# sash-a/hrl_pybullet_envs

Measured on AMD Instinct MI355X. Metric: env-steps/sec, AntGatherBulletEnv-v0 @4096 envs, 1/2/4/8 MI355X, higher is better.
Workload: dtype f32; 1 GPU; AntGatherBulletEnv-v0, 4096 envs per GPU, U(-1,1) actions pre-generated on device, auto-reset, max_episode_steps 2000; envs_per_gpu=4096, global_envs=4096, parallelism=one GPU, one process, no collective

## Files before the change

### hrl_pybullet_envs_amd/csrc/step_core.h

```cpp
#pragma once
#include <math.h>
#include <stdint.h>

#include <utility>

#ifdef HRL_EMU
#define HRL_DEV inline
#define HRL_PIN_VGPR(x) ((void)0)
#define HRL_PIN_INT(x) ((void)0)
#define HRL_PIN_SCALAR(x) ((void)0)
#else
#define HRL_DEV __device__ __forceinline__
#define HRL_PIN_VGPR(x) asm volatile("" : "+v"(x))
#define HRL_PIN_INT(x) asm volatile("" : "+s"(x))
#define HRL_PIN_SCALAR(x) asm volatile("" : "+s"(x))
#endif


namespace hrl {

constexpr int NJ = 8;
constexpr int MAXC = 12;
constexpr int MAXR = 44;
constexpr int MAXB = NJ + MAXC;
// ... 1315 lines not shown
        }
        x.reg(lane).ud = d < 6 ? v : 0.f;
        if (lane < 16) L.ustar[lane] = d < 6 ? v : 0.f;
        float ax_[3], ay_[3], az_[3];
        quat_axes(q[3], q[4], q[5], q[6], ax_, ay_, az_);
#pragma unroll
        for (int k = 0; k < 3; ++k) { L.XYZ[k] = ax_[k]; L.XYZ[3 + k] = ay_[k]; L.XYZ[6 + k] = az_[k]; }
    });
    int nC = 0;
    auto corner = [&](int lane, bool on, int f, int item) {
        CornerHit h; h.ok = false; h.dist = 0.f; h.n[0] = h.n[1] = 0.f; h.n[2] = 1.f; h.c[0] = h.c[1] = h.c[2] = 0.f; h.surf = f;
        if (on) {
            float sx = (lane & 1) ? he : -he, sy = (lane & 2) ? he : -he, sz = (lane & 4) ? he : -he;
#pragma unroll
            for (int k = 0; k < 3; ++k) h.c[k] = fma_(sz, L.XYZ[6 + k], fma_(sy, L.XYZ[3 + k], sx * L.XYZ[k]));
            const float p[3] = {q[0] + h.c[0], q[1] + h.c[1], q[2] + h.c[2]};
            if (item >= 0) {
                const float ix = L.items[2 * item], iy = L.items[2 * item + 1];
                const float lo[3] = {ix - ITEM_HALF, iy - ITEM_HALF, ITEM_Z - ITEM_HALF}, hi[3] = {ix + ITEM_HALF, iy + ITEM_HALF, ITEM_Z + ITEM_HALF};
                h.dist = sphere_vs_box(p, 0.f, lo, hi, h.n); h.surf = surf_item(item);
            } else if (f == 0) h.dist = p[2] - c.ground_z;
            else {
                h.n[0] = L.planes[f - 1][0]; h.n[1] = L.planes[f - 1][1]; h.n[2] = L.planes[f - 1][2];
                h.dist = dot3(h.n, p) - L.planes[f - 1][3];
            }
            h.ok = h.dist < c.cdist;
        }
        return h;
    };
    auto keep = [&](int base) {
        return [&L, base](int, int rank, const CornerHit &h) {
            const int i = base + rank;
            if (i < MAXC) {
#pragma unroll
                for (int k = 0; k < 3; ++k) { L.cr[i][k] = h.c[k]; L.cdir[0][i][k] = h.n[k]; }
                L.cdist_[i] = h.dist; L.csurf[i] = h.surf;
            }
        };
    };
    {
        int cnt = x.each_compact([&](int lane) { return corner(lane, (lane >> 3) < 1 + c.n_planes, lane >> 3, -1); }, keep(nC), [&](int, const CornerHit &) {});
        nC += cnt;
        if (nC > cap) nC = cap;
    }
    if (items_on) {
        const float R = 0.35f * 1.7320508f + ITEM_HALF + c.cdist + 0.02f;
        unsigned long long near = x.each_ballot([&](int lane) {
            return (lane < c.n_food + c.n_poison) & (fabsf(q[0] - L.items[2 * lane]) < R) & (fabsf(q[1] - L.items[2 * lane + 1]) < R);
        });
        const unsigned long long near0 = near;
        while (near) {
            int it[4];
#pragma unroll
            for (int k = 0; k < 4; ++k) {
                it[k] = -1;
                if (near) { it[k] = (int)__builtin_ctzll(near); near &= near - 1; }
            }
            int cnt = x.each_compact(
                [&](int lane) {
                    const int slot = lane >> 3;
                    const int item = slot == 0 ? it[0] : (slot == 1 ? it[1] : (slot == 2 ? it[2] : (slot == 3 ? it[3] : -1)));
                    return corner(lane, item >= 0, 0, item);
                },
                keep(nC), [&](int, const CornerHit &) {});
            nC += cnt;
            if (nC > cap) nC = cap;
        }
        x.refresh();
#pragma unroll 1
        for (int ib = 0; ib < 64; ib += 32) {
        unsigned near32 = (unsigned)(near0 >> ib);
        while (near32) {
            const unsigned group = near32;
#pragma unroll
            for (int k = 0; k < 8; ++k) near32 &= near32 - 1;
            int cnt = x.each_compact(
                [&](int lane) {
                    const int slot = lane >> 3;
                    unsigned m = group;
#pragma unroll
                    for (int k = 0; k < 7; ++k) m = k < slot ? (m & (m - 1)) : m;
                    const int item = m ? ib + (int)__builtin_ctz(m) : -1;
                    CornerHit h; h.ok = false; h.dist = 0.f; h.n[0] = h.n[1] = 0.f; h.n[2] = 1.f; h.c[0] = h.c[1] = h.c[2] = 0.f; h.surf = 0;
                    if (item >= 0) {
                        const float ix = L.items[2 * item], iy = L.items[2 * item + 1];
                        const float pc[3] = {(lane & 1) ? ix + ITEM_HALF : ix - ITEM_HALF, (lane & 2) ? iy + ITEM_HALF : iy - ITEM_HALF,
                                             (lane & 4) ? ITEM_Z + ITEM_HALF : ITEM_Z - ITEM_HALF};
                        const float d[3] = {pc[0] - q[0], pc[1] - q[1], pc[2] - q[2]};
                        const float l[3] = {dot3(d, &L.XYZ[0]), dot3(d, &L.XYZ[3]), dot3(d, &L.XYZ[6])}, blo[3] = {-he, -he, -he}, bhi[3] = {he, he, he};
                        float nl[3];
                        h.dist = sphere_vs_box(l, 0.f, blo, bhi, nl); h.surf = surf_item(item);
#pragma unroll
                        for (int k = 0; k < 3; ++k) {
                            const float nw = fma_(nl[2], L.XYZ[6 + k], fma_(nl[1], L.XYZ[3 + k], nl[0] * L.XYZ[k]));
                            h.n[k] = -nw; h.c[k] = fma_(-h.dist, nw, d[k]);
                        }
                        h.ok = h.dist < c.cdist;
                    }
                    return h;
                },
                keep(nC), [&](int, const CornerHit &) {});
            nC += cnt;
            if (nC > cap) nC = cap;
        }
        }
    }
    x.each([&](int lane) {
        if (lane < nC) { const float n[3] = {L.cdir[0][lane][0], L.cdir[0][lane][1], L.cdir[0][lane][2]}; store_contact_frame(L, lane, n); }
    });
    x.each([&](int lane) {
        LaneRegs &g = x.reg(lane);
        g.fn = -1;
        if (lane >= 3 * nC) return;
        const int ci = lane < nC ? lane : (lane - nC) >> 1, which = lane < nC ? 0 : 1 + ((lane - nC) & 1);
        const float r[3] = {L.cr[ci][0], L.cr[ci][1], L.cr[ci][2]};
        const float d[3] = {L.cdir[which][ci][0], L.cdir[which][ci][1], L.cdir[which][ci][2]};
        float J[6], B[16];
#pragma unroll
        for (int k = 0; k < 16; ++k) B[k] = 0.f;
        cross3(J, r, d);
#pragma unroll
        for (int k = 0; k < 3; ++k) { J[3 + k] = d[k]; B[k] = J[k] / I; B[3 + k] = d[k] / m; }
        const float dist = L.cdist_[ci];
#pragma unroll
        for (int k = 0; k < 6; ++k) g.Jb[k] = J[k];
        g.Jh = 0.f; g.Ja = 0.f; g.jslot = 6 | (6 << 8); g.mu = which == 0 ? 0.f : c.mu;
#pragma unroll
        for (int k = 0; k < 16; ++k) L.Bt[lane][k] = B[k];
        g.bias = which == 0 ? (dist > 0.f ? dist : c.erp_c * dist) * c.inv_h : 0.f;
        g.fn = which == 0 ? -1 : ci; g.lam = 0.f; g.lo = 0.f; g.hi = which == 0 ? 1e30f : 0.f;
    });
    pgs_solve<MAXC>(x, c, 0, nC, false, false);
    x.each([&](int lane) { if (lane < 16) L.u[lane] = x.reg(lane).ud; });
    x.stamp(10);
    x.each([&](int lane) { phase_integrate(c, L, q, qn, lane); });
    x.stamp(11);
    return nC;
}


HRL_DEV void quat_to_rpy(const float *qq, float *rpy) {
    float x = qq[0], y = qq[1], z = qq[2], w = qq[3];
    float sarg = -2.f * (x * z - w * y);
    const float hp = 1.5707963267948966f;
    if (sarg <= -0.99999f) { rpy[0] = 0.f; rpy[1] = -hp; rpy[2] = 2.f * atan2_spec(x, -y); }
    else if (sarg >= 0.99999f) { rpy[0] = 0.f; rpy[1] = hp; rpy[2] = 2.f * atan2_spec(-x, y); }
    else {
        float sqx = x * x, sqy = y * y, sqz = z * z, sqw = w * w;
        rpy[0] = atan2_spec(2.f * (y * z + w * x), ((sqw - sqx) - sqy) + sqz);
        rpy[1] = asin_spec(sarg);
        rpy[2] = atan2_spec(2.f * (x * y + w * z), ((sqw + sqx) - sqy) - sqz);
    }
}
HRL_DEV float wrap_angle(float a) {
    const float two_pi = 6.283185307179586f, pi = 3.141592653589793f;
    if (!(fabsf(a) < two_pi)) a = fmodf(a, two_pi);
    if (a < 0.f) a += two_pi;
    if (a >= two_pi) a -= two_pi;
    if (a > pi) a = a - two_pi;
    if (a < -pi) a = a + two_pi;
    return a;
}
HRL_DEV int quadrant(float x, float y) {
    if (x >= 0.f && y >= 0.f) return 1;
    if (x >= 0.f && y <= 0.f) return 4;
    if (x <= 0.f && y >= 0.f) return 2;
    if (x <= 0.f && y <= 0.f) return 3;
    return -1;
}
HRL_DEV bool inf_intersection(float x1, float y1, float x2, float y2, float x3, float y3, float x4, float y4, float *px, float *py) {
    float d = (x1 - x2) * (y3 - y4) - (y1 - y2) * (x3 - x4);
    if (d == 0.f) return false;
    *px = ((x1 * y2 - y1 * x2) * (x3 - x4) - (x1 - x2) * (x3 * y4 - y3 * x4)) / d;
    *py = ((x1 * y2 - y1 * x2) * (y3 - y4) - (y1 - y2) * (x3 * y4 - y3 * x4)) / d;
    return true;
}
HRL_DEV int orientation(float px, float py, float qx, float qy, float rx, float ry) {
    float val = ((qy - py) * (rx - qx)) - ((qx - px) * (ry - qy));
    return val > 0.f ? 1 : (val < 0.f ? 2 : 0);
}
HRL_DEV bool on_segment(float px, float py, float qx, float qy, float rx, float ry) {
    return (qx <= fmaxf(px, rx)) && (qx >= fminf(px, rx)) && (qy <= fmaxf(py, ry)) && (qy >= fminf(py, ry));
}
HRL_DEV bool segment_intersection(float p1x, float p1y, float q1x, float q1y, float p2x, float p2y, float q2x, float q2y) {
    int o1 = orientation(p1x, p1y, q1x, q1y, p2x, p2y), o2 = orientation(p1x, p1y, q1x, q1y, q2x, q2y);
    int o3 = orientation(p2x, p2y, q2x, q2y, p1x, p1y), o4 = orientation(p2x, p2y, q2x, q2y, q1x, q1y);
    if (o1 != o2 && o3 != o4) return true;
    if (o1 == 0 && on_segment(p1x, p1y, p2x, p2y, q1x, q1y)) return true;
    if (o2 == 0 && on_segment(p1x, p1y, q2x, q2y, q1x, q1y)) return true;
    if (o3 == 0 && on_segment(p2x, p2y, p1x, p1y, q2x, q2y)) return true;
    if (o4 == 0 && on_segment(p2x, p2y, q1x, q1y, q2x, q2y)) return true;
    return false;
}
HRL_DEV void maze_line(int l, float *a) {
    const float T[7][4] = {{5, 9, -5, 9}, {5, 9, 5, -9}, {-5, -9, -5, 9}, {-5, -9, 5, -9}, {1, 2, 1, -2}, {-5, -2, -5, 2}, {-5, -2, 1, -2}};
#pragma unroll
    for (int k = 0; k < 4; ++k) {
        float v = T[0][k];
#pragma unroll
        for (int i = 1; i < 7; ++i) v = (l == i) ? T[i][k] : v;
        a[k] = v;
    }
}

HRL_DEV void flag_goal(const DevCfg &c, uint32_t ep, uint32_t k, float *gx, float *gy) {
    for (uint32_t a = 0; a < 64; ++a) {
        uint32_t r[4];
        philox4x32(c, 0, ep, (4u << 16) | k, a, r);
        *gx = -c.flag_size / 2.f + c.flag_size * u01(r[0]); *gy = -c.flag_size / 2.f + c.flag_size * u01(r[1]);
        if (!(sqrtf(*gx * *gx + *gy * *gy) < 0.5f)) break;
    }
}

HRL_DEV void flag_close_goal(const DevCfg &c, long long env, uint32_t ep, uint32_t k, float rx, float ry, float *gx, float *gy) {
    const float wb = c.flag_size / 2.f, half = c.flag_mtd / 2.f;
    for (uint32_t a = 0; a < 64; ++a) {
        uint32_t r[4];
        philox4x32(c, env, ep, (5u << 16) | (k & 0xffffu), a, r);
        *gx = (c.tol + (half - c.tol) * u01(r[0])) * ((r[2] & 1u) ? 1.f : -1.f) + rx;
        *gy = (c.tol + (half - c.tol) * u01(r[1])) * ((r[3] & 1u) ? 1.f : -1.f) + ry;
        if (-wb < *gx && *gx < wb && -wb < *gy && *gy < wb) break;
    }
}

HRL_DEV void flag_set_target_state(WaveLds &L, float gx, float gy, float px, float py) {
    const float dx = gx - px, dy = gy - py, nrm = sqrtf(dx * dx + dy * dy);
    L.items[HRL_FLAG_START_OFF] = px; L.items[HRL_FLAG_START_OFF + 1] = py; L.items[HRL_FLAG_SQDIST_OFF] = nrm * nrm;
}

HRL_DEV float wall_sensor_bin(const DevCfg &c, float rx, float ry, float yaw, int i, bool arena) {
    const float half_pi = 1.5707963267948966f;
    float phi;
    if (c.span_is_2pi) phi = half_pi + yaw + ((float)(i + 1) / (float)c.n_bins) * c.sensor_span;
    else phi = half_pi + yaw + ((float)i / (float)(c.n_bins - 1)) * c.sensor_span;
    const float svx = rx + c.sensor_range * cos_spec(phi), svy = ry + c.sensor_range * sin_spec(phi);
    const int sq = quadrant(svx - rx, svy - ry);
    float best = 0.f;
    for (int l = 0; l < (arena ? 4 : 7); ++l) {
        float a[4], px, py;
        if (arena) {
            const float hx = c.world_sx / 2.f, hy = c.world_sy / 2.f;
            a[0] = l < 2 ? hx : -hx; a[1] = l < 2 ? hy : -hy;
            a[2] = (l == 0 || l == 2) ? -hx : hx; a[3] = (l == 0) ? hy : ((l == 1) ? -hy : ((l == 2) ? hy : -hy));
        } else maze_line(l, a);
        if (!inf_intersection(rx, ry, svx, svy, a[0], a[1], a[2], a[3], &px, &py)) continue;
        const float ddx = rx - px, ddy = ry - py, dist = sqrtf(ddx * ddx + ddy * ddy);
        if (dist > c.sensor_range) continue;
        if (sq != quadrant(px - rx, py - ry)) continue;
        const float val = 1.f - dist / c.sensor_range;
        if (val > best) best = val;
    }
    return best;
}

template <class X>
HRL_DEV void maze_target(X &x, const DevCfg &c, WaveLds &L, float *tx, float *ty) {
    const unsigned ti = (unsigned)x.uniform(L.aux[3]);
    const int k = ti < (unsigned)HRL_MAX_TARGETS ? (int)ti : 0;
    *tx = c.targets[k][0]; *ty = c.targets[k][1];
}

template <int KIND>
HRL_DEV void phase_calc_state(const DevCfg &c, WaveLds &L, int lane, bool use_feet, bool with_centroid, float mtx, float mty) {
    const float *qp = L.st, *qv = L.st + 15;
    float rpy[3];
    quat_to_rpy(qp + 3, rpy);
    float tx = c.walk_tx, ty = c.walk_ty;
    if (KIND == 5) {
        if (c.flag_mtd > 0.f || c.flag_manual) { tx = L.items[0]; ty = L.items[1]; }
        else flag_goal(c, (uint32_t)L.aux[2], (uint32_t)L.aux[3] & 0xffffu, &tx, &ty);
    }
    if (KIND == 2 || KIND == 4) { tx = mtx; ty = mty; }
    if (KIND == 5) { L.red[4] = tx; L.red[5] = ty; }
    float cx = qp[0], cy = qp[1];
    if (with_centroid) {
        float sx = 0.f, sy = 0.f;
#pragma unroll
        for (int l = 0; l < 4; ++l) {
            sx += (0.5f * L.ph[l][0] + 0.5f * (L.ph[l][0] + L.pa[l][0])) + 0.5f * (L.pa[l][0] + L.tip[l][0]);
            sy += (0.5f * L.ph[l][1] + 0.5f * (L.ph[l][1] + L.pa[l][1])) + 0.5f * (L.pa[l][1] + L.tip[l][1]);
        }
        const float np_ = (float)(13 + c.centroid_n_static);
        cx = ((13.f * qp[0] + sx) + c.centroid_sx) / np_;
        cy = ((13.f * qp[1] + sy) + c.centroid_sy) / np_;
    }
    const float dx = tx - cx, dy = ty - cy;
    float sin_ang = 0.f, cos_ang = 0.f, wtd = 0.f;
    if (KIND != 1) {
        const float theta = atan2_spec(dy, dx), ang = theta - rpy[2];
        wtd = sqrtf(dy * dy + dx * dx); sin_ang = sin_spec(ang); cos_ang = cos_spec(ang);
    }
    const float cs = cos_spec(-rpy[2]), sn = sin_spec(-rpy[2]);
    const float vx = cs * qv[0] - sn * qv[1], vy = sn * qv[0] + cs * qv[1], vz = qv[2];
    int nlim = 0;
    float mine = 0.f;
#pragma unroll
    for (int j = 0; j < NJ; ++j) {
        const float rel = (qp[7 + j] - c.jmid[j]) * c.jscale[j];
        if (fabsf(rel) > 0.99f) ++nlim;
        mine = (lane == 8 + 2 * j) ? rel : mine;
        mine = (lane == 9 + 2 * j) ? 0.1f * qv[6 + j] : mine;
    }
    mine = (lane == 0) ? qp[2] - L.st[30] : mine;
    mine = (lane == 1) ? sin_ang : mine;
    mine = (lane == 2) ? cos_ang : mine;
    mine = (lane == 3) ? 0.3f * vx : mine;
    mine = (lane == 4) ? 0.3f * vy : mine;
    mine = (lane == 5) ? 0.3f * vz : mine;
    mine = (lane == 6) ? rpy[0] : mine;
    mine = (lane == 7) ? rpy[1] : mine;
    if (lane >= 24 && lane < 28) {
        const int l = lane - 24;
        mine = (use_feet && ((L.aux[1] >> (28 + l)) & 1)) ? 1.f : 0.f;
    }
    if (lane < 28) L.s28[lane] = clampf(mine, -5.f, 5.f);
    L.scal[3] = wtd; L.scal[4] = rpy[2]; L.scal[5] = (float)nlim; L.scal[6] = cx; L.scal[7] = cy;
}

HRL_DEV void respawn_item(const DevCfg &c, long long env, uint32_t index, uint32_t purpose, int item, float ax, float ay, float *px, float *py) {
    const float sxw = c.world_sx - 1.f, syw = c.world_sy - 1.f;
    for (uint32_t a = 0; a < 64; ++a) {
        uint32_t r[4];
        philox4x32(c, env, index, (purpose << 16) | (uint32_t)item, a, r);
        *px = u01(r[0]) * sxw - sxw / 2.f; *py = u01(r[1]) * syw - syw / 2.f;
        const float dx = ax - *px, dy = ay - *py;
        if (!(sqrtf(dx * dx + dy * dy) < c.spacing)) break;
    }
}

HRL_DEV void phase_items(const DevCfg &c, WaveLds &L, int lane, long long env, bool pickups, int n_contacts) {
    const int n = c.n_food + c.n_poison;
    float rew = 0.f, bin = -1.f, inten = 0.f;
    if (lane < n) {
        const float rx = L.st[0], ry = L.st[1], yaw = L.scal[4];
        float ix = L.items[2 * lane], iy = L.items[2 * lane + 1];
        float dx = ix - rx, dy = iy - ry, d2 = dx * dx + dy * dy;
        if (pickups && c.coll_dist > 0.f && d2 < c.coll_dist) {
            rew = lane < c.n_food ? 1.f : -1.f;
            if (c.respawn) respawn_item(c, env, (uint32_t)L.aux[1], 0u, lane, rx, ry, &ix, &iy);
            else { ix = 100.f; iy = 0.f; }
            L.items[2 * lane] = ix; L.items[2 * lane + 1] = iy;
            dx = ix - rx; dy = iy - ry; d2 = dx * dx + dy * dy;
        }
        if (!c.use_sensor) inten = d2;
        else if (d2 != d2) bin = -2.f;
        else if (!(d2 > c.sensor_range)) {
            const float half_span = c.sensor_span * 0.5f, bin_res = c.sensor_span / (float)c.n_bins;
            const float angle = wrap_angle(atan2_spec(iy - ry, ix - rx) - yaw);
            if (fabsf(angle) <= half_span) {
                int b = (int)((angle + half_span) / bin_res);
                if (b >= c.n_bins) b = c.n_bins - 1;
                bin = (float)b; inten = 1.0f - d2 / c.sensor_range;
            }
        }
        if (pickups && !(c.coll_dist > 0.f)) {
            int hits = 0;
            for (int i = 0; i < n_contacts; ++i) hits += L.csurf[i] == surf_item(lane) ? 1 : 0;
            rew = (lane < c.n_food ? 1.f : -1.f) * (float)hits;
        }
    }
    L.irew[lane] = rew; L.ibin[lane] = bin; L.iint[lane] = inten;
}

HRL_DEV void phase_items_contact_move(const DevCfg &c, WaveLds &L, int lane, long long env) {
    if (lane >= c.n_food + c.n_poison) return;
    const int hits = (int)fabsf(L.irew[lane]);
    if (hits > 0) {
        float ix = 100.f, iy = 0.f;
        if (c.respawn) respawn_item(c, env, (uint32_t)L.aux[1], 0u, lane | ((hits - 1) << c.item_shift), L.st[0], L.st[1], &ix, &iy);
        L.items[2 * lane] = ix; L.items[2 * lane + 1] = iy;
    }
}

template <int KIND>
HRL_DEV void phase_pack_obs(const DevCfg &c, WaveLds &L, int lane , float mtx, float mty) {
    if (lane >= c.obs_dim) return;
    float v = 0.f;
    if (KIND == 0) v = L.st[lane];
    else if (KIND == 5) {
        if (lane < 28) v = L.s28[lane];
        else v = wall_sensor_bin(c, L.st[0], L.st[1], L.scal[4], lane - 28, true);
    }
    else if (KIND == 4) {
        if (lane < 29) v = L.st[lane];
        else if (lane < 29 + c.n_bins) v = wall_sensor_bin(c, L.st[0], L.st[1], L.scal[4], lane - 29, false);
        else if (lane == 29 + 3 * c.n_bins) v = (float)L.aux[0] * 0.001f;
    }
    else if (KIND == 3) {
        if (lane < 8) v = L.s28[lane];
    } else if (lane < 26) v = L.s28[lane == 0 ? 0 : lane + 2];
    const int nb = (KIND == 3) ? 8 : 26;
    if ((KIND == 1 || KIND == 3) && lane >= nb && c.use_sensor) {
        const int b = lane - nb, type = b / c.n_bins, bin = b - type * c.n_bins;
        const int k0 = type ? c.n_food : 0, k1 = type ? c.n_food + c.n_poison : c.n_food;
        float best = 0.f;
        bool bad = false;
#pragma unroll
        for (int k = 0; k < 16; ++k) {
            const bool mine = (k >= k0) & (k < k1);
            const bool take = mine & (L.ibin[k] == (float)bin) & (L.iint[k] > best);
            best = take ? L.iint[k] : best;
            bad = bad | (mine & (L.ibin[k] == -2.f));
        }
#pragma unroll 1
        for (int k = 16; k < k1; ++k) {
            const bool mine = k >= k0;
            const bool take = mine & (L.ibin[k] == (float)bin) & (L.iint[k] > best);
            best = take ? L.iint[k] : best;
            bad = bad | (mine & (L.ibin[k] == -2.f));
        }
        v = bad ? __builtin_nanf("") : best;
    }
    if ((KIND == 1 || KIND == 3) && lane >= nb && !c.use_sensor) {
        const int mf = c.n_food < c.n_bins ? c.n_food : c.n_bins;
        const int b = lane - nb, type = b >= 2 * mf, bb = type ? b - 2 * mf : b, want = bb >> 1, comp = bb & 1;
        const int k0 = type ? c.n_food : 0, k1 = type ? c.n_food + c.n_poison : c.n_food;
        bool bad = false;
        for (int i = k0; i < k1; ++i) {
            int rank = 0;
            for (int j = k0; j < k1; ++j) rank += (L.iint[j] < L.iint[i] || (L.iint[j] == L.iint[i] && j < i)) ? 1 : 0;
            if (rank == want) v = L.items[2 * i + comp];
            bad = bad | (L.iint[i] != L.iint[i]);
        }
        if (bad && want < (k1 - k0)) v = __builtin_nanf("");
    }
    if (KIND == 2 && lane >= 26) {
        const float rx = L.st[0], ry = L.st[1], yaw = L.scal[4];
        const float tx = mtx, ty = mty;
        const int ntar = c.sense_target ? c.n_bins : 2;
        if (lane < 26 + ntar) {
            const int i = lane - 26;
            if (!c.sense_target) {
                const float vx = tx - rx, vy = ty - ry;
                if (c.target_encoding == 0) { const float n = sqrtf(vx * vx + vy * vy); v = i == 0 ? vx / n : vy / n; }
                else { const float a = atan2_spec(vy, vx) - yaw; v = i == 0 ? sin_spec(a) : cos_spec(a); }
            } else {
                const float wtd = L.scal[3];
                bool vis = !(wtd > c.sensor_range);
                for (int l = 4; l < 7 && vis; ++l) { float a[4]; maze_line(l, a); if (segment_intersection(rx, ry, tx, ty, a[0], a[1], a[2], a[3])) vis = false; }
                if (vis) {
                    const float angle = wrap_angle(atan2_spec(ty - ry, tx - rx) - yaw), half_span = c.sensor_span * 0.5f;
                    if (fabsf(angle) <= half_span) {
                        int b = (int)((angle + half_span) / (c.sensor_span / (float)c.n_bins));
                        if (b >= c.n_bins) b = c.n_bins - 1;
                        if (b == i) v = 1.0f - wtd / c.sensor_range;
                    }
                }
            }
        } else v = wall_sensor_bin(c, rx, ry, yaw, lane - 26 - ntar, false);
    }
    L.obs[lane] = v;
    if (!isfinite(v)) L.flags[0] = 1;
}

HRL_DEV void phase_point_state(const DevCfg &c, WaveLds &L, int lane) {
    const float *qp = L.st, *qv = L.st + 15;
    float rpy[3];
    quat_to_rpy(qp + 3, rpy);
    const float theta = atan2_spec(0.f - qp[1], 0.f - qp[0]), a = theta - rpy[2];
    const float cs = cos_spec(-rpy[2]), sn = sin_spec(-rpy[2]);
    const float vx = cs * qv[0] - sn * qv[1], vy = sn * qv[0] + cs * qv[1], vz = qv[2];
    float mine = qp[2] - 1.f;
    mine = (lane == 1) ? sin_spec(a) : mine;
    mine = (lane == 2) ? cos_spec(a) : mine;
    mine = (lane == 3) ? 0.3f * vx : mine;
    mine = (lane == 4) ? 0.3f * vy : mine;
    mine = (lane == 5) ? 0.3f * vz : mine;
    mine = (lane == 6) ? rpy[0] : mine;
    mine = (lane == 7) ? rpy[1] : mine;
    if (lane < 8) L.s28[lane] = mine;
    L.scal[3] = 0.f; L.scal[4] = rpy[2]; L.scal[5] = 0.f;
    (void)c;
}

template <int KIND, class X>
HRL_DEV void compute_obs(X &x, const DevCfg &c, long long env, bool step_mode, int n_contacts = 0) {
    WaveLds &L = x.lds();
    const bool centroid = (KIND == 0 || KIND == 2 || KIND == 4 || KIND == 5);
    if (centroid) {
        x.each([&](int lane) { if (lane < 16) L.q[0][lane] = lane < 15 ? L.st[lane] : 0.f; });
        x.each([&](int lane) { phase_kin_ankle<true>(c, L, x.reg(lane), L.q[0], lane); });
    }
    float mtx = 0.f, mty = 0.f;
    if (KIND == 2 || KIND == 4) maze_target(x, c, L, &mtx, &mty);
    x.each([&](int lane) { if (lane < 4) L.flags[lane] = 0; });
    if (KIND == 3) x.each([&](int lane) { phase_point_state(c, L, lane); });
    else {
        const bool feet = KIND == 2 || KIND == 5;
        x.each([&](int lane) { phase_calc_state<KIND>(c, L, lane, feet, centroid, mtx, mty); });
    }
    x.stamp(21);
    if (KIND == 1 || KIND == 3) x.each([&](int lane) { phase_items(c, L, lane, env, step_mode, n_contacts); });
    x.stamp(22);
#pragma unroll 1
    for (int o = 0; o < c.obs_dim; o += 64) x.each([&](int lane) { phase_pack_obs<KIND>(c, L, lane + o, mtx, mty); });
    if ((KIND == 1 || KIND == 3) && step_mode && !(c.coll_dist > 0.f)) x.each([&](int lane) { phase_items_contact_move(c, L, lane, env); });
}


template <int KIND, class X>
HRL_DEV void reset_env(X &x, const DevCfg &c, long long env) {
    WaveLds &L = x.lds();
    float ptx = c.walk_tx, pty = c.walk_ty;
    if (KIND == 2 || KIND == 4 || KIND == 5) {
        if (x.uniform(L.aux[2]) > 0) {
            if (KIND == 5) {
                if (c.flag_mtd > 0.f || c.flag_manual) { ptx = L.items[0]; pty = L.items[1]; }
                else flag_goal(c, (uint32_t)L.aux[2], (uint32_t)L.aux[3] & 0xffffu, &ptx, &pty);
            } else maze_target(x, c, L, &ptx, &pty);
        }
        x.each([](int) {});
    }
    x.each([&](int lane) {
        const uint32_t ep = (uint32_t)L.aux[2];
        if (lane < 32) {
            float v = 0.f;
            if (lane == 6) v = 1.f;
            if (KIND == 3) { if (lane == 2) v = 0.5f; if (lane == 30) v = 1.f; }
            else {
                float z0 = 0.75f;
                if (KIND == 2 || KIND == 4 || KIND == 5) { z0 = c.start_pos[2]; if (lane == 0) v = c.start_pos[0]; if (lane == 1) v = c.start_pos[1]; }
                if (lane == 2 || lane == 30) v = z0;
                if (lane >= 7 && lane < 15) {
                    const int j = lane - 7;
                    uint32_t r[4];
                    philox4x32(c, env, ep, (2u << 16) | (uint32_t)(j >> 2), 0u, r);
                    const uint32_t rr = (j & 3) == 0 ? r[0] : ((j & 3) == 1 ? r[1] : ((j & 3) == 2 ? r[2] : r[3]));
                    v = -0.1f + 0.2f * u01(rr);
                }
            }
            L.st[lane] = v;
        } else if (KIND == 1 || KIND == 3) {
            const int i = lane - 32;
            if (i < 16) {
                float px = 0.f, py = 0.f;
                if (i < c.n_food + c.n_poison) respawn_item(c, env, ep, 1u, i, 0.f, 0.f, &px, &py);
                L.items[2 * i] = px; L.items[2 * i + 1] = py;
            }
        } else if (KIND == 5 && c.flag_path_on) {
            const int w = lane - 32;
            if (c.flag_manual) {
                if (w == 0) L.items[0] = ptx;
                if (w == 1) L.items[1] = pty;
                if (w >= HRL_FLAG_PENDING_OFF) L.items[w] = 0.f;
            } else {
                float gx = 0.f, gy = 0.f;
                if (w == 0) {
                    if (c.flag_mtd > 0.f) flag_close_goal(c, env, ep + 1u, 1u, c.start_pos[0], c.start_pos[1], &gx, &gy);
                    else flag_goal(c, ep + 1u, 1u, &gx, &gy);
                    flag_set_target_state(L, gx, gy, c.start_pos[0], c.start_pos[1]);
                    L.items[0] = c.flag_mtd > 0.f ? gx : 0.f; L.items[1] = c.flag_mtd > 0.f ? gy : 0.f;
                    L.items[HRL_FLAG_SQDIST_OFF + 1] = 0.f;
                } else if (w >= HRL_FLAG_PENDING_OFF) L.items[w] = 0.f;
            }
        }
        if (lane < 16) L.u[lane] = 0.f;
        if (lane < 8) L.tau[lane] = 0.f;
        if (lane == 63 && KIND == 5) L.aux[3] = (int)((c.flag_manual ? 0u : 1u) | ((uint32_t)L.aux[3] & 0x7fff0000u));
        if (lane == 63 && (KIND == 2 || KIND == 4)) {
            uint32_t r[4];
            philox4x32(c, env, ep, (3u << 16), 0u, r);
            L.aux[3] = (int)(r[0] % (uint32_t)c.n_targets);
        }
    });
    if ((KIND == 1 || KIND == 3 || KIND == 5) && c.items_stride > 32)
        x.each([&](int lane) {
            const uint32_t ep = (uint32_t)L.aux[2];
            const int i = 16 + lane;
            if (i < HRL_MAX_ITEMS) {
                float px = 0.f, py = 0.f;
                if ((KIND == 1 || KIND == 3) && i < c.n_food + c.n_poison) respawn_item(c, env, ep, 1u, i, 0.f, 0.f, &px, &py);
                L.items[2 * i] = px; L.items[2 * i + 1] = py;
            }
        });
    x.each([&](int lane) {
        if (lane == 0) L.aux[0] = 0;
        if (lane == 1 && (KIND == 2 || KIND == 5)) L.aux[1] = L.aux[1] & 0x0fffffff;
        if (lane == 2) L.aux[2] = L.aux[2] + 1;
    });
    compute_obs<KIND>(x, c, env, false);
    x.each([&](int lane) {
        if (lane != 31) return;
        float pot = 0.f;
        if (KIND == 0) pot = -L.scal[3] / c.dt;
        if (KIND == 2 || KIND == 4 || KIND == 5) {
            float cx = L.scal[6], cy = L.scal[7];
            if (KIND != 5) { const float np_ = (float)(13 + c.centroid_n_static); cx = cx - (13.f * c.start_pos[0]) / np_; cy = cy - (13.f * c.start_pos[1]) / np_; }
            const float dx = ptx - cx, dy = pty - cy;
            pot = -sqrtf(dy * dy + dx * dx) / c.dt;
        }
        L.st[31] = pot;
    });
}

template <class X>
HRL_DEV void load_env(X &x, const DevBufs &b, const DevCfg &c, int e, bool with_actions) {
    WaveLds &L = x.lds();
    x.each([&](int lane) {
        if (lane < 32) L.st[lane] = b.state[(size_t)e * 32 + lane];
        else { const float v = b.items ? b.items[(size_t)e * c.items_stride + (lane - 32)] : 0.f; L.items[lane - 32] = v; L.items0[lane - 32] = v; }
#pragma unroll 1
        for (int o = 32; o < c.items_stride; o += 64)
            if (o + lane < c.items_stride) L.items[o + lane] = b.items ? b.items[(size_t)e * c.items_stride + (o + lane)] : 0.f;
        if (lane < 4) L.aux[lane] = b.aux[(size_t)e * 4 + lane];
        if (lane < 8) L.act[lane] = (with_actions && lane < c.act_dim) ? b.actions[(size_t)e * c.act_dim + lane] : 0.f;
        if (lane >= 8 && lane < 16) { L.jlim[0][lane - 8] = c.jlo[lane - 8]; L.jlim[1][lane - 8] = c.jhi[lane - 8]; }
        if (lane >= 16 && lane < 32) { const int f = (lane - 16) >> 2, k = lane & 3; L.planes[f][k] = k < 3 ? c.plane_n[f][k] : c.plane_d[f]; }
    });
}
template <class X>
HRL_DEV void store_env(X &x, const DevBufs &b, const DevCfg &c, int e) {
    WaveLds &L = x.lds();
    x.each([&](int lane) {
        if (lane < 32) b.state[(size_t)e * 32 + lane] = L.st[lane];
        else if (b.items) {
            const float v = L.items[lane - 32];
            if (float_bits(v) != float_bits(L.items0[lane - 32])) b.items[(size_t)e * c.items_stride + (lane - 32)] = v;
        }
#pragma unroll 1
        for (int o = 32; o < c.items_stride; o += 64)
            if (b.items && o + lane < c.items_stride) b.items[(size_t)e * c.items_stride + (o + lane)] = L.items[o + lane];
        if (lane < 4) b.aux[(size_t)e * 4 + lane] = L.aux[lane];
        if (lane < c.obs_dim) b.obs[(size_t)e * c.obs_dim + lane] = L.obs[lane];
#pragma unroll 1
        for (int o = 64; o < c.obs_dim; o += 64)
            if (o + lane < c.obs_dim) b.obs[(size_t)e * c.obs_dim + (o + lane)] = L.obs[o + lane];
    });
}

template <int KIND, class X>
HRL_DEV void reset_entry(X &x, const DevBufs &b, const DevCfg &c, int e) {
    if (b.mask && !b.mask[e]) return;
    load_env(x, b, c, e, false);
    reset_env<KIND>(x, c, c.env_id_offset + e);
    store_env(x, b, c, e);
}

template <int KIND, class X>
HRL_DEV void observe_entry(X &x, const DevBufs &b, const DevCfg &c, int e) {
    if (b.mask && !b.mask[e]) return;
    WaveLds &L = x.lds();
    load_env(x, b, c, e, false);
    compute_obs<KIND>(x, c, c.env_id_offset + e, false);
    x.each([&](int lane) {
#pragma unroll 1
        for (int o = 0; o < c.obs_dim; o += 64)
            if (o + lane < c.obs_dim) b.obs[(size_t)e * c.obs_dim + (o + lane)] = L.obs[o + lane];
    });
}

template <class X>
HRL_DEV void set_goals_entry(X &x, const DevBufs &b, const DevCfg &c, int e, const float *goals_xy, int n_goals, uint8_t *ok) {
    if (b.mask && !b.mask[e]) return;
    WaveLds &L = x.lds();
    const long long env = c.env_id_offset + e;
    load_env(x, b, c, e, false);
    if (n_goals > 0) {
        x.each([&](int lane) {
#pragma unroll 1
            for (int w = lane; w < c.items_stride; w += 64)
                if (w >= HRL_FLAG_PENDING_OFF) {
                    const int k = (w - HRL_FLAG_PENDING_OFF) >> 1, comp = w & 1;
                    L.items[w] = k < n_goals ? goals_xy[((size_t)e * n_goals + k) * 2 + comp] : 0.f;
                }
            if (lane == 63) L.aux[3] = (int)(((uint32_t)n_goals & 0xffffu) | ((uint32_t)L.aux[3] & 0xffff0000u));
        });
    }
    x.each([&](int lane) {
        if (lane != 0) return;
        const uint32_t a3 = (uint32_t)L.aux[3];
        uint32_t cur = a3 & 0xffffu;
        int good = 1;
        float gx = L.items[0], gy = L.items[1];
        if (c.flag_mtd > 0.f) {
            cur = (cur + 1u) & 0xffffu;
            flag_close_goal(c, env, (uint32_t)L.aux[2], cur, L.st[0], L.st[1], &gx, &gy);
        } else if (!c.flag_manual) {
            if (cur >= (uint32_t)c.flag_max_targets) good = 0; else cur += 1u;
        } else if (cur == 0u) good = 0;
        else { cur -= 1u; gx = L.items[HRL_FLAG_PENDING_OFF + 2 * cur]; gy = L.items[HRL_FLAG_PENDING_OFF + 1 + 2 * cur]; }
        if (good) {
            if (!c.flag_manual && !(c.flag_mtd > 0.f)) flag_goal(c, (uint32_t)L.aux[2], cur, &gx, &gy);
            else { L.items[0] = gx; L.items[1] = gy; }
            if (c.flag_path_on) flag_set_target_state(L, gx, gy, L.st[0], L.st[1]);
            L.aux[3] = (int)(cur | (a3 & 0x7fff0000u));
        }
        if (ok) ok[e] = (uint8_t)good;
    });
    compute_obs<5>(x, c, env, false);
    store_env(x, b, c, e);
}

template <int KIND, class X>
HRL_DEV void write_contacts(X &x, const DevCfg &c, float *rec, const float *q0, int n_contacts, int nL) {
    const WaveLds &L = x.lds();
    x.each([&](int lane) {
        float v0 = 0.f, v1 = 0.f, v2 = 0.f, v3 = 0.f;
        const int nR = nL + 3 * n_contacts;
        if (lane == 0) { v0 = (float)n_contacts; v1 = (float)nL; v2 = (float)nR; v3 = c.h; }
        else if (lane < 3) {
            for (int k = 0; k < nL; ++k) {
                const int j = (L.ljoint[k] & 7) - 4 * (lane - 1);
                const float f = L.lsign[k] * L.lamf[k];
                v0 = j == 0 ? f : v0; v1 = j == 1 ? f : v1; v2 = j == 2 ? f : v2; v3 = j == 3 ? f : v3;
            }
        } else if (lane == 3) {
            int held = 0, neg = 0;
            for (int k = 0; k < nL; ++k) { const int bit = 1 << (L.ljoint[k] & 7); held |= bit; neg |= L.lsign[k] < 0.f ? bit : 0; }
            v0 = (float)held; v1 = (float)neg;
        } else {
            const int m = lane - 4, i = m / 5, w = m - 5 * i;
            if (i < n_contacts) {
                if (w == 0) { v0 = L.cr[i][0] + q0[0]; v1 = L.cr[i][1] + q0[1]; v2 = L.cr[i][2] + q0[2]; v3 = L.cdist_[i]; }
                else if (w < 4) {
                    const int d = w - 1;
                    v0 = L.cdir[d][i][0]; v1 = L.cdir[d][i][1]; v2 = L.cdir[d][i][2];
                    v3 = L.lamf[d == 0 ? nL + i : nL + n_contacts + 2 * i + (d - 1)];
                } else {
                    v0 = (float)L.csurf[i];
                    v1 = KIND == 3 ? 0.f : (float)L.clink[i]; v2 = KIND == 3 ? -1.f : (float)L.clink2[i]; v3 = KIND == 3 ? c.mu : L.cmu[i];
                }
            }
        }
#ifdef HRL_EMU
        float *o = rec + 4 * lane;
        o[0] = v0; o[1] = v1; o[2] = v2; o[3] = v3;
#else
        reinterpret_cast<float4 *>(rec)[lane] = make_float4(v0, v1, v2, v3);
#endif
    });
}

template <int KIND, class X>
HRL_DEV void step_entry(X &x, const DevBufs &b, const DevCfg &c, int e) {
    WaveLds &L = x.lds();
    const bool on = e < c.n_envs;
    if (on) {
        load_env(x, b, c, e, true);
        x.each([&](int lane) {
            if (lane < 16) {
                L.q[0][lane] = lane < 15 ? L.st[lane] : 0.f;
                const int src = lane < 3 ? 15 + 3 + lane : (lane < 6 ? 15 + lane - 3 : 15 + lane);
                L.u[lane] = lane < 14 ? L.st[src] : 0.f;
            }
            if (lane >= 16 && lane < 24) {
                const int j = lane - 16;
                if (KIND == 3) {
                    const float n = sqrtf(L.act[0] * L.act[0] + L.act[1] * L.act[1]);
                    L.tau[j] = j < 2 ? L.act[j] / n * c.point_force : 0.f;
                } else L.tau[j] = c.torque_scale * clampf(L.act[j], -1.f, 1.f);
            }
        });
    }
    x.stamp(12);
    int qi = 0, n_contacts = 0;
    int rows_acc = 0;
    const bool items_on = (KIND == 1 || KIND == 3) && c.item_collision != 0;
    HRL_PIN_INT(qi);
    const int slot = x.slot();
    if constexpr (KIND == 3) {
#pragma unroll 1
        for (int s = 0; s < c.nsub; ++s) {
            x.priority(slot + s);
            n_contacts = point_substep(x, c, qi, items_on);
            rows_acc += 3 * n_contacts;
            qi ^= 1;
            HRL_PIN_INT(qi);
        }
    } else {
        x.each([&](int lane) { if (lane == 0) L.on = on ? 1 : 0; });
        if (!on)
            x.each([&](int lane) {
                if (lane < 16) {
                    const float v = lane == 2 ? 1e3f : (lane == 6 ? 1.f : 0.f);
                    L.q[0][lane] = v; L.q[1][lane] = v; L.u[lane] = 0.f;
                }
                if (lane < 8) { L.tau[lane] = 0.f; L.jlim[0][lane] = -1e3f; L.jlim[1][lane] = 1e3f; }
                L.items[lane] = 1e6f; L.items[64 + lane] = 1e6f;
                if (lane >= 16 && lane < 32) L.planes[(lane - 16) >> 2][lane & 3] = (lane & 3) == 2 ? 1.f : ((lane & 3) == 3 ? -1e6f : 0.f);
            });
        x.group_sync();
#pragma unroll 1
        for (int s = 0; s < c.nsub; ++s) {
            x.priority(slot + s);
            HRL_PIN_VGPR(qi);
#ifndef HRL_ABLATE_GROUP
            ant_group_block(x, c, qi);
#endif
#ifndef HRL_ABLATE_CONTACTS
            ant_contact_duty(x, c, qi, items_on);
#endif
            x.stamp(16);
            x.group_sync();
            x.stamp(17);
#ifndef HRL_ABLATE_ENV
            if (on) rows_acc += ant_env_block(x, c, qi);
#endif
            x.group_sync();
            x.stamp(19);
            qi ^= 1;
        }
        if (on) n_contacts = x.uniform(L.nC);
    }
    if (!on) return;
    int eo = e;
    HRL_PIN_VGPR(eo);
    const long long env = c.env_id_offset + eo;
    if (b.contacts)
        write_contacts<KIND>(x, c, b.contacts + (size_t)eo * HRL_CONTACTS_STRIDE, L.q[qi ^ 1], n_contacts, KIND == 3 ? 0 : x.uniform(L.nL));
    x.each([&](int lane) {
        if (lane < 15) L.st[lane] = L.q[qi][lane];
        if (lane >= 16 && lane < 30) {
            const int k = lane - 16;
            L.st[15 + k] = k < 3 ? L.u[3 + k] : (k < 6 ? L.u[k - 3] : L.u[k]);
        }
    });
    x.stamp(13);
    compute_obs<KIND>(x, c, env, true, n_contacts);
    x.stamp(14);
    x.each([&](int lane) {
        float rew = 0.f, food = 0.f, dead = 0.f;
        int done = 0;
        if (KIND == 1 || KIND == 3) {
            for (int k = 0; k < c.n_food + c.n_poison; ++k) food += L.irew[k];
            float alive = 1.f;
            if (KIND == 1) alive = (L.obs[0] + L.st[30] > 0.26f) ? 1.f : -1.f;
            done = (alive < 0.f) || L.flags[0];
            dead = alive < 0.f ? c.dying_cost : 0.f;
            rew = food + dead;
        } else if (KIND == 0) {
            const float alive = L.st[2] > 0.26f ? 1.f : -1.f;
            done = (alive < 0.f) || L.flags[0];
            const float pot = -L.scal[3] / c.dt, progress = pot - L.st[31];
            rew = ((alive + progress) + -0.1f * L.scal[5]) + 0.f;
            food = alive; dead = progress;
            L.red[0] = pot;
        } else if (KIND == 5) {
            const float alive = (L.s28[0] + L.st[30] > 0.26f) ? 1.f : -1.f;
            int idone = alive < 0.f;
            for (int i = 0; i < 28; ++i) if (!isfinite(L.s28[i])) idone = 1;
            const float wtd = L.scal[3], pot = -wtd / c.dt, progress = pot - L.st[31];
            L.red[0] = pot;
            int steps = ((L.aux[3] >> 16) & 0x7fff) + 1, rewarded = (L.aux[3] >> 31) & 1, cur = L.aux[3] & 0xffff, retarget = 0;
            const bool close = c.flag_mtd > 0.f, listed = c.flag_manual && !close;
            const int step_cur = listed ? -1 : 1;
            auto more = [&]() { return close ? true : (listed ? cur > 0 : cur < c.flag_max_targets); };
            float e1 = 0.f, e2 = 0.f;
            for (int j = 0; j < NJ; ++j) { const float a = L.act[j]; e1 += fabsf(a * L.s28[9 + 2 * j]); e2 += a * a; }
            const float electricity = c.w_elec * (e1 / NJ) + c.w_stall * (e2 / NJ);
            rew = ((((alive + progress) + electricity) + c.w_jal * L.scal[5]) + 0.f) * c.flag_w_env;
            food = alive; dead = progress;
            if (c.flag_path_on) {
                const float gsx = L.items[HRL_FLAG_START_OFF], gsy = L.items[HRL_FLAG_START_OFF + 1];
                const float path = ((L.st[0] - gsx) * (L.red[4] - gsx) + (L.st[1] - gsy) * (L.red[5] - gsy)) / L.items[HRL_FLAG_SQDIST_OFF];
                rew = rew + path * c.flag_w_path;
            }
            rew = rew + (-wtd) * c.flag_w_dist;
            done = idone;
            if (wtd < c.tol) {
                if (!rewarded) { rew += c.flag_goal_rew; rewarded = 1; }
                if (c.flag_switch) {
                    if (more()) { cur += step_cur; rewarded = 0; steps = 0; retarget = 1; } else done = 1;
                }
            }
            if (c.flag_timeout > 0 && c.flag_timeout <= steps) {
                if (more()) { cur += step_cur; rewarded = 0; steps = 0; retarget = 1; } else done = 1;
            }
            if (steps > 0x7fff) steps = 0x7fff;
            L.flags[4] = (int)(((uint32_t)cur & 0xffffu) | ((uint32_t)steps << 16) | ((uint32_t)rewarded << 31));
            L.flags[3] = retarget;
        } else if (KIND == 4) {
            const float alive = L.st[2] > 0.26f ? 1.f : -1.f;
            int idone = alive < 0.f;
            for (int i = 0; i < 29; ++i) if (!isfinite(L.st[i])) idone = 1;
            const float wtd = L.scal[3], pot = -wtd / c.dt, progress = pot - L.st[31];
            const float inner = ((alive + progress) + -0.1f * L.scal[5]) + 0.f;
            food = alive; dead = progress;
            rew = inner * c.inner_rew_weight;
            done = idone;
            if (wtd < c.tol) { rew += 1.f; done = 1; }
            L.red[0] = pot;
        } else {
            const float alive = (L.s28[0] + L.st[30] > 0.26f) ? 1.f : -1.f;
            int idone = alive < 0.f;
            for (int i = 0; i < 28; ++i) if (!isfinite(L.s28[i])) idone = 1;
            const float wtd = L.scal[3], pot = -wtd / c.dt, progress = pot - L.st[31];
            float e1 = 0.f, e2 = 0.f;
            for (int j = 0; j < NJ; ++j) { const float a = L.act[j]; e1 += fabsf(a * L.s28[9 + 2 * j]); e2 += a * a; }
            const float electricity = c.w_elec * (e1 / NJ) + c.w_stall * (e2 / NJ);
            const float inner = (((alive + progress) + electricity) + c.w_jal * L.scal[5]) + 0.f;
            food = alive; dead = progress;
            rew = inner * c.inner_rew_weight;
            done = idone;
            const int t = L.aux[0] + 1;
            if (wtd < c.tol) { if (c.done_at_target || (!c.done_at_target && t == c.max_steps - 1)) { rew += 1.f; done = 1; } }
            if (t == c.max_steps - 1) done = 1;
            if (c.targ_dist_rew && done) rew -= wtd;
            L.red[0] = pot;
        }
        const int t_ep = L.aux[0] + 1;
        int trunc = 0;
        if (c.max_episode_steps > 0 && t_ep >= c.max_episode_steps) { trunc = !done; done = 1; }
        L.scal[0] = rew; L.scal[1] = food; L.scal[2] = dead; L.flags[1] = done; L.flags[2] = trunc;
        L.red[1] = L.st[29] + rew; L.red[2] = (float)t_ep;
    });
    x.each([&](int lane) {
        if (lane == 0) {
            L.aux[0] = L.aux[0] + 1; b.reward[eo] = L.scal[0]; b.done[eo] = (uint8_t)L.flags[1];
            if (b.truncated) b.truncated[eo] = (uint8_t)L.flags[2];
            if (b.rows) b.rows[eo] += rows_acc;
        }
        if (lane == 1) {
            int a1 = L.aux[1] + 1;
            if (KIND == 2 || KIND == 5) {
                int bits = 0;
#pragma unroll
                for (int l = 0; l < 4; ++l) bits |= ((L.gtouch[2 + 3 * l] | L.gtouch[3 + 3 * l]) & 1) << l;
                a1 = (a1 & 0x0fffffff) | (bits << 28);
            }
            L.aux[1] = a1;
        }
        if (lane == 2 && (KIND == 0 || KIND == 2 || KIND == 4 || KIND == 5)) L.st[31] = L.red[0];
        if (lane == 3) L.st[29] = L.red[1];
        if (lane == 8 && KIND == 5) L.aux[3] = L.flags[4];
        if (lane == 9 && KIND == 5 && L.flags[3]) {
            float gx, gy;
            if (c.flag_mtd > 0.f) flag_close_goal(c, env, (uint32_t)L.aux[2], (uint32_t)L.flags[4] & 0xffffu, L.st[0], L.st[1], &gx, &gy);
            else if (c.flag_manual) {
                const int top = L.flags[4] & 0xffff;
                gx = L.items[HRL_FLAG_PENDING_OFF + 2 * top]; gy = L.items[HRL_FLAG_PENDING_OFF + 1 + 2 * top];
            } else flag_goal(c, (uint32_t)L.aux[2], (uint32_t)L.flags[4] & 0xffffu, &gx, &gy);
            if (c.flag_mtd > 0.f || c.flag_manual) { L.items[0] = gx; L.items[1] = gy; }
            if (c.flag_path_on) flag_set_target_state(L, gx, gy, L.st[0], L.st[1]);
        }
        if (lane >= 4 && lane < 8) {
            const int k = lane - 4;
            b.info[(size_t)eo * 4 + k] = k == 0 ? L.scal[1] : (k == 1 ? L.scal[2] : (k == 2 ? L.red[1] : L.red[2]));
        }
    });
    const int done_u = x.uniform(L.flags[1]);
    if constexpr (KIND == 5) {
        const int retarget_u = x.uniform(L.flags[3]);
        if (retarget_u) compute_obs<KIND>(x, c, env, true);
        if (b.goal)
            x.each([&](int lane) {
                if (lane < HRL_GOAL_STRIDE)
                    b.goal[(size_t)eo * HRL_GOAL_STRIDE + lane] = lane == 0 ? L.red[4] : (lane == 1 ? L.red[5] : (lane == 2 ? (retarget_u ? 1.f : 0.f) : (float)((L.aux[3] >> 16) & 0x7fff)));
            });
    }
    if (done_u && b.final_obs)
        x.each([&](int lane) {
#pragma unroll 1
            for (int o = 0; o < c.obs_dim; o += 64)
                if (o + lane < c.obs_dim) b.final_obs[(size_t)eo * c.obs_dim + (o + lane)] = L.obs[o + lane];
        });
    if (done_u && c.auto_reset) reset_env<KIND>(x, c, env);
    store_env(x, b, c, eo);
    x.stamp(15);
    x.flush_stamps(b);
}

template <class X>
HRL_DEV void step_dispatch(X &x, const DevBufs &b, const DevCfg &c, int e) {
    switch (c.kind) {
        case 0: step_entry<0>(x, b, c, e); break;
        case 1: step_entry<1>(x, b, c, e); break;
        case 2: step_entry<2>(x, b, c, e); break;
        case 3: step_entry<3>(x, b, c, e); break;
        case 4: step_entry<4>(x, b, c, e); break;
        default: step_entry<5>(x, b, c, e); break;
    }
// ... 26 lines not shown
```

Baseline: 77.57 million env-steps/s.

## Distribute ant-gather observation phases across group waves for packed env processing

For the ant-gather kind, the state-record copy moves into the last substep. Calc-state and item sensing are then computed cooperatively across the wave group: one wave computes calc-state for all four envs (16 lanes each) and another computes item sensing, followed by a group sync. This replaces the per-env serial compute_obs phases, which leave most lanes idle. It adds a group barrier, recomputes yaw per lane, and keeps inactive waves alive until the sync.

```diff
diff --git a/hrl_pybullet_envs_amd/csrc/step_core.h b/hrl_pybullet_envs_amd/csrc/step_core.h
--- a/hrl_pybullet_envs_amd/csrc/step_core.h
+++ b/hrl_pybullet_envs_amd/csrc/step_core.h
@@ -1491,6 +1491,14 @@
         rpy[2] = atan2_spec(2.f * (x * y + w * z), ((sqw + sqx) - sqy) - sqz);
     }
 }
+HRL_DEV float quat_yaw(const float *qq) {
+    float x = qq[0], y = qq[1], z = qq[2], w = qq[3];
+    float sarg = -2.f * (x * z - w * y);
+    if (sarg <= -0.99999f) return 2.f * atan2_spec(x, -y);
+    if (sarg >= 0.99999f) return 2.f * atan2_spec(-x, y);
+    float sqx = x * x, sqy = y * y, sqz = z * z, sqw = w * w;
+    return atan2_spec(2.f * (x * y + w * z), ((sqw + sqx) - sqy) - sqz);
+}
 HRL_DEV float wrap_angle(float a) {
     const float two_pi = 6.283185307179586f, pi = 3.141592653589793f;
     if (!(fabsf(a) < two_pi)) a = fmodf(a, two_pi);
@@ -1599,8 +1607,14 @@
     *tx = c.targets[k][0]; *ty = c.targets[k][1];
 }
 
+struct CalcState {
+    float head[8];
+    float rel[NJ], jv[NJ];
+    float wtd, yaw, cx, cy;
+    int nlim;
+};
 template <int KIND>
-HRL_DEV void phase_calc_state(const DevCfg &c, WaveLds &L, int lane, bool use_feet, bool with_centroid, float mtx, float mty) {
+HRL_DEV void calc_state_values(const DevCfg &c, WaveLds &L, bool with_centroid, float mtx, float mty, CalcState &o) {
     const float *qp = L.st, *qv = L.st + 15;
     float rpy[3];
     quat_to_rpy(qp + 3, rpy);
@@ -1632,28 +1646,55 @@
     const float cs = cos_spec(-rpy[2]), sn = sin_spec(-rpy[2]);
     const float vx = cs * qv[0] - sn * qv[1], vy = sn * qv[0] + cs * qv[1], vz = qv[2];
     int nlim = 0;
-    float mine = 0.f;
 #pragma unroll
     for (int j = 0; j < NJ; ++j) {
         const float rel = (qp[7 + j] - c.jmid[j]) * c.jscale[j];
         if (fabsf(rel) > 0.99f) ++nlim;
-        mine = (lane == 8 + 2 * j) ? rel : mine;
-        mine = (lane == 9 + 2 * j) ? 0.1f * qv[6 + j] : mine;
-    }
-    mine = (lane == 0) ? qp[2] - L.st[30] : mine;
-    mine = (lane == 1) ? sin_ang : mine;
-    mine = (lane == 2) ? cos_ang : mine;
-    mine = (lane == 3) ? 0.3f * vx : mine;
-    mine = (lane == 4) ? 0.3f * vy : mine;
-    mine = (lane == 5) ? 0.3f * vz : mine;
-    mine = (lane == 6) ? rpy[0] : mine;
-    mine = (lane == 7) ? rpy[1] : mine;
-    if (lane >= 24 && lane < 28) {
-        const int l = lane - 24;
+        o.rel[j] = rel; o.jv[j] = 0.1f * qv[6 + j];
+    }
+    o.head[0] = qp[2] - L.st[30]; o.head[1] = sin_ang; o.head[2] = cos_ang;
+    o.head[3] = 0.3f * vx; o.head[4] = 0.3f * vy; o.head[5] = 0.3f * vz;
+    o.head[6] = rpy[0]; o.head[7] = rpy[1];
+    o.wtd = wtd; o.yaw = rpy[2]; o.cx = cx; o.cy = cy; o.nlim = nlim;
+}
+HRL_DEV float calc_state_entry(const WaveLds &L, const CalcState &v, int k, bool use_feet) {
+    float mine = 0.f;
+#pragma unroll
+    for (int j = 0; j < NJ; ++j) {
+        mine = (k == 8 + 2 * j) ? v.rel[j] : mine;
+        mine = (k == 9 + 2 * j) ? v.jv[j] : mine;
+    }
+#pragma unroll
+    for (int i = 0; i < 8; ++i) mine = (k == i) ? v.head[i] : mine;
+    if (k >= 24 && k < 28) {
+        const int l = k - 24;
         mine = (use_feet && ((L.aux[1] >> (28 + l)) & 1)) ? 1.f : 0.f;
     }
-    if (lane < 28) L.s28[lane] = clampf(mine, -5.f, 5.f);
-    L.scal[3] = wtd; L.scal[4] = rpy[2]; L.scal[5] = (float)nlim; L.scal[6] = cx; L.scal[7] = cy;
+    return clampf(mine, -5.f, 5.f);
+}
+HRL_DEV void calc_state_scal(WaveLds &L, const CalcState &v) {
+    L.scal[3] = v.wtd; L.scal[4] = v.yaw; L.scal[5] = (float)v.nlim; L.scal[6] = v.cx; L.scal[7] = v.cy;
+}
+template <int KIND>
+HRL_DEV void phase_calc_state(const DevCfg &c, WaveLds &L, int lane, bool use_feet, bool with_centroid, float mtx, float mty) {
+    CalcState v;
+    calc_state_values<KIND>(c, L, with_centroid, mtx, mty, v);
+    if (lane < 28) L.s28[lane] = calc_state_entry(L, v, lane, use_feet);
+    calc_state_scal(L, v);
+}
+template <int KIND, class X>
+HRL_DEV void calc_state_group(X &x, const DevCfg &c, bool use_feet) {
+    x.each([&](int lane) {
+        WaveLds &L = x.lds(lane >> 4);
+        if (!L.on) return;
+        const int k = lane & 15;
+        CalcState v;
+        calc_state_values<KIND>(c, L, false, 0.f, 0.f, v);
+        L.s28[k] = calc_state_entry(L, v, k, use_feet);
+        if (k + 16 < 28) L.s28[k + 16] = calc_state_entry(L, v, k + 16, use_feet);
+        calc_state_scal(L, v);
+        if (k < 4) L.flags[k] = 0;
+    });
 }
 
 HRL_DEV void respawn_item(const DevCfg &c, long long env, uint32_t index, uint32_t purpose, int item, float ax, float ay, float *px, float *py) {
@@ -1667,11 +1708,11 @@
     }
 }
 
-HRL_DEV void phase_items(const DevCfg &c, WaveLds &L, int lane, long long env, bool pickups, int n_contacts) {
+HRL_DEV void phase_items(const DevCfg &c, WaveLds &L, int lane , long long env, bool pickups, int n_contacts, float yaw) {
     const int n = c.n_food + c.n_poison;
     float rew = 0.f, bin = -1.f, inten = 0.f;
     if (lane < n) {
-        const float rx = L.st[0], ry = L.st[1], yaw = L.scal[4];
+        const float rx = L.st[0], ry = L.st[1];
         float ix = L.items[2 * lane], iy = L.items[2 * lane + 1];
         float dx = ix - rx, dy = iy - ry, d2 = dx * dx + dy * dy;
         if (pickups && c.coll_dist > 0.f && d2 < c.coll_dist) {
@@ -1699,6 +1740,17 @@
         }
     }
     L.irew[lane] = rew; L.ibin[lane] = bin; L.iint[lane] = inten;
+}
+template <class X>
+HRL_DEV void items_group(X &x, const DevCfg &c, int e0) {
+    const int n = c.n_food + c.n_poison;
+#pragma unroll 1
+    for (int base = 0; base == 0 || base < n; base += 16)
+        x.each([&](int lane) {
+            WaveLds &L = x.lds(lane >> 4);
+            if (!L.on) return;
+            phase_items(c, L, base + (lane & 15), c.env_id_offset + (e0 + (lane >> 4)), true, L.nC, quat_yaw(L.st + 3));
+        });
 }
 
 HRL_DEV void phase_items_contact_move(const DevCfg &c, WaveLds &L, int lane, long long env) {
@@ -1813,6 +1865,14 @@
 }
 
 template <int KIND, class X>
+HRL_DEV void pack_obs(X &x, const DevCfg &c, long long env, bool step_mode, float mtx, float mty) {
+    WaveLds &L = x.lds();
+#pragma unroll 1
+    for (int o = 0; o < c.obs_dim; o += 64) x.each([&](int lane) { phase_pack_obs<KIND>(c, L, lane + o, mtx, mty); });
+    if ((KIND == 1 || KIND == 3) && step_mode && !(c.coll_dist > 0.f)) x.each([&](int lane) { phase_items_contact_move(c, L, lane, env); });
+}
+
+template <int KIND, class X>
 HRL_DEV void compute_obs(X &x, const DevCfg &c, long long env, bool step_mode, int n_contacts = 0) {
     WaveLds &L = x.lds();
     const bool centroid = (KIND == 0 || KIND == 2 || KIND == 4 || KIND == 5);
@@ -1829,11 +1889,9 @@
         x.each([&](int lane) { phase_calc_state<KIND>(c, L, lane, feet, centroid, mtx, mty); });
     }
     x.stamp(21);
-    if (KIND == 1 || KIND == 3) x.each([&](int lane) { phase_items(c, L, lane, env, step_mode, n_contacts); });
+    if (KIND == 1 || KIND == 3) x.each([&](int lane) { phase_items(c, L, lane, env, step_mode, n_contacts, L.scal[4]); });
     x.stamp(22);
-#pragma unroll 1
-    for (int o = 0; o < c.obs_dim; o += 64) x.each([&](int lane) { phase_pack_obs<KIND>(c, L, lane + o, mtx, mty); });
-    if ((KIND == 1 || KIND == 3) && step_mode && !(c.coll_dist > 0.f)) x.each([&](int lane) { phase_items_contact_move(c, L, lane, env); });
+    pack_obs<KIND>(x, c, env, step_mode, mtx, mty);
 }
 
 
@@ -2070,6 +2128,18 @@
     });
 }
 
+template <class X>
+HRL_DEV void packed_record(X &x, int qi) {
+    WaveLds &L = x.lds();
+    x.each([&](int lane) {
+        if (lane < 15) L.st[lane] = L.q[qi][lane];
+        if (lane >= 16 && lane < 30) {
+            const int k = lane - 16;
+            L.st[15 + k] = k < 3 ? L.u[3 + k] : (k < 6 ? L.u[k - 3] : L.u[k]);
+        }
+    });
+}
+
 template <int KIND, class X>
 HRL_DEV void step_entry(X &x, const DevBufs &b, const DevCfg &c, int e) {
     WaveLds &L = x.lds();
@@ -2095,6 +2165,7 @@
     int qi = 0, n_contacts = 0;
     int rows_acc = 0;
     const bool items_on = (KIND == 1 || KIND == 3) && c.item_collision != 0;
+    constexpr bool packed = KIND == 1;
     HRL_PIN_INT(qi);
     const int slot = x.slot();
     if constexpr (KIND == 3) {
@@ -2135,27 +2206,33 @@
 #ifndef HRL_ABLATE_ENV
             if (on) rows_acc += ant_env_block(x, c, qi);
 #endif
+            if (packed && on && s == c.nsub - 1) packed_record(x, qi ^ 1);
             x.group_sync();
             x.stamp(19);
             qi ^= 1;
         }
         if (on) n_contacts = x.uniform(L.nC);
     }
-    if (!on) return;
+    if (!packed && !on) return;
     int eo = e;
     HRL_PIN_VGPR(eo);
     const long long env = c.env_id_offset + eo;
-    if (b.contacts)
+    if (on && b.contacts)
         write_contacts<KIND>(x, c, b.contacts + (size_t)eo * HRL_CONTACTS_STRIDE, L.q[qi ^ 1], n_contacts, KIND == 3 ? 0 : x.uniform(L.nL));
-    x.each([&](int lane) {
-        if (lane < 15) L.st[lane] = L.q[qi][lane];
-        if (lane >= 16 && lane < 30) {
-            const int k = lane - 16;
-            L.st[15 + k] = k < 3 ? L.u[3 + k] : (k < 6 ? L.u[k - 3] : L.u[k]);
-        }
-    });
-    x.stamp(13);
-    compute_obs<KIND>(x, c, env, true, n_contacts);
+    if constexpr (packed) {
+        x.stamp(13);
+        const int w = x.wave_index();
+        if (w == 1) { calc_state_group<KIND>(x, c, false); x.stamp(21); }
+        if (w == 2) { items_group(x, c, eo - w); x.stamp(22); }
+        x.group_sync();
+        x.stamp(23);
+        if (!on) return;
+        pack_obs<KIND>(x, c, env, true, 0.f, 0.f);
+    } else {
+        packed_record(x, qi);
+        x.stamp(13);
+        compute_obs<KIND>(x, c, env, true, n_contacts);
+    }
     x.stamp(14);
     x.each([&](int lane) {
         float rew = 0.f, food = 0.f, dead = 0.f;
```

Result: no change. 78.30 million env-steps/s, median of 6 (+0.9%).
